# wenzhang-dev/bitcaskDB

Hardware: AMD Instinct MI355X
Metric: WAL record decode+CRC GiB/s (device-resident), 4 KiB values, 1/2/4/8 MI355X (higher is better)
Workload: dtype u8; 1 GPU; config B: 1073743514 B WAL segment per GPU, NsSize 20, 100 B keys, 4 KiB values, device-resident decode+CRC+record parse; seg_bytes=1073743514, records=253846, fragments=286402, parallelism=one independent segment per GPU x1

## Files before the change

bitcaskdb_amd/csrc/bcw_decode.hip:

```cpp
#include <hip/hip_runtime.h>

#include <cstdint>

#include "bcw_internal.h"
#include "bcw_parse.h"

namespace bcw {

enum { M_FIRST_BAD = 0,
       M_NE = 1,
       M_NFRAGS = 4, M_DONE_CRC = 5,
       M_T_CRC0 = 10, M_T_FIN = 11,
       M_ABORT = 12,
       M_BAD_CRC = 14,
       M_BAD_TYPE = 15 };

__device__ __forceinline__ uint32_t rotl32(uint32_t x, int r) { return (x << r) | (x >> (32 - r)); }

__device__ __forceinline__ void read_header(const uint8_t* __restrict__ seg, uint64_t seg_len, uint64_t off,
                                            uint32_t& crc, uint32_t& len, uint32_t& type) {
  const uint64_t a = off & ~3ull;
  uint32_t w0, w1, w2;
  if (a + 12 <= seg_len) {
    const uint32_t* q = reinterpret_cast<const uint32_t*>(seg + a);
// ... 42 lines not shown
__device__ __forceinline__ uint32_t wave_max_scan(uint32_t v, uint32_t) {
  return wave_scan_z(v, [](uint32_t x, uint32_t y) { return max(x, y); });
}
__device__ __forceinline__ uint32_t wave_or_scan(uint32_t v, uint32_t) {
  return wave_scan_z(v, [](uint32_t x, uint32_t y) { return x | y; });
}
__device__ __forceinline__ uint32_t wave_add_scan(uint32_t v, uint32_t) {
  return wave_scan_z(v, [](uint32_t x, uint32_t y) { return x + y; });
}

__device__ __forceinline__ uint32_t wg256_excl_scan(uint32_t v, uint32_t* sm4, uint32_t& total) {
  const uint32_t lane = threadIdx.x & 63u, wave = threadIdx.x >> 6;
  const uint32_t incl = wave_incl_scan_u32(v, lane);
  if (lane == 63) sm4[wave] = incl;
  __syncthreads();
  uint32_t base = 0;
  for (uint32_t k = 0; k < wave; ++k) base += sm4[k];
  total = sm4[0] + sm4[1] + sm4[2] + sm4[3];
  __syncthreads();
  return base + incl - v;
}

struct Spin {
  uint64_t t0 = 0;
  uint64_t lim = 20000000ull;
  __device__ __forceinline__ bool go(uint64_t* misc, uint32_t site) {
    const uint64_t t = wall_clock64();
    if (t0 == 0) t0 = t;
    if (t - t0 < lim &&
        __hip_atomic_load(&misc[M_ABORT], __ATOMIC_RELAXED, __HIP_MEMORY_SCOPE_AGENT) == 0ull) {
      __builtin_amdgcn_s_sleep(1);
      return true;
    }
    atomicMax(reinterpret_cast<unsigned long long*>(&misc[M_ABORT]), (unsigned long long)site);
    return false;
  }
};

constexpr int kChaseHold = 64;
constexpr uint64_t kLbAgg = 1, kLbInc = 2, kLbMask = (1ull << 38) - 1;
constexpr int kDirect = BCW_CHASE_DIRECT_MAX;

template <typename V>
__device__ __forceinline__ uint32_t chase_block(const uint8_t* __restrict__ seg, uint64_t seg_len, uint64_t boff,
                                                uint32_t bufsize, V&& visit, uint32_t h = 0, uint32_t n = 0) {
  while (h + kHdr <= bufsize) {
    uint32_t crc, len, type;
    read_header(seg, seg_len, boff + h, crc, len, type);
    const uint32_t start = h + kHdr;
    if (len > bufsize - start) len = bufsize - start;
    visit(n, start, len, crc, type);
    ++n;
    h = start + len;
  }
  return n;
}

constexpr uint32_t kRecUsual = 1u << 20, kRecAdj = 1u << 21;
__device__ __forceinline__ uint32_t check_word(uint32_t crc, uint32_t ic) { return ~rotl32(crc - 0xa282ead8u, 15) ^ ic; }
__device__ __forceinline__ void put_frag_J(Frag* __restrict__ frags, uint4* __restrict__ srec, uint64_t g,
                                           uint64_t frag_cap, uint32_t b, uint64_t boff, uint32_t start_len,
                                           uint32_t J, uint32_t type, bool adj) {
  if (g >= frag_cap) return;
  *reinterpret_cast<uint4*>(frags + g) = make_uint4(b, start_len, J, type & 0xffu);
  const uint64_t gs = boff + (start_len & 0xffffu), ge = gs + (start_len >> 16);
  const uint32_t cb = (uint32_t)(gs / kSChunk), ce = (uint32_t)(ge / kSChunk);
  const uint32_t pa = (uint32_t)(gs % kSChunk), pb = (uint32_t)(ge % kSChunk);
  const bool usual = adj && cb < ce && pb <= (uint32_t)kSChunk - 8u;
  const uint32_t e = pb + 4u, K = ((e % kSPiece) + 3u) >> 2, Lfull = e / kSPiece + (K == (uint32_t)kSPW ? 1u : 0u);
  srec[g] = make_uint4(ce, cb, J, pb | pa << 10 | (usual ? kRecUsual : 0u) | (adj ? kRecAdj : 0u) | Lfull << 22 |
                                      (K & 3u) << 29);
}
__device__ __forceinline__ void put_frag(Frag* __restrict__ frags, uint4* __restrict__ srec, uint64_t g,
                                         uint64_t frag_cap, uint32_t b, uint64_t boff, uint32_t start, uint32_t len,
                                         uint32_t crc, uint32_t type, const uint32_t* __restrict__ initc, bool adj) {
  put_frag_J(frags, srec, g, frag_cap, b, boff, start | (len << 16), check_word(crc, initc[len]), type, adj);
}

constexpr uint32_t kSumHasE = 1u << 16;

struct ClassW {
  uint64_t pw;
  uint64_t pp0, pp1;
  uint64_t p8;
  __device__ __forceinline__ uint64_t weight(uint32_t y) const {
    return (uint64_t)(65536 + 256 * (int64_t)(int8_t)(uint8_t)(pw >> (8u * y)));
  }
  __device__ __forceinline__ uint64_t prefix(uint32_t y) const {
    const uint64_t f = (y < 4u ? pp0 : pp1) >> (16u * (y & 3u));
    return (uint64_t)(65536 * (int64_t)y + 256 * (int64_t)(int16_t)(uint16_t)f);
  }
  __device__ __forceinline__ uint32_t classes_below(double x) const {
    uint32_t n = 0;
#pragma unroll
    for (uint32_t k = 1; k < 8; ++k) n += (double)prefix(k) <= x ? 1u : 0u;
    return n;
  }
};
__device__ __forceinline__ uint64_t div_floor(uint64_t a, uint64_t b, double rb) {
  uint64_t q = (uint64_t)((double)a * rb);
  while (q * b > a) --q;
  while ((q + 1) * b <= a) ++q;
  return q;
}
struct WavePart {
  ClassW cw;
  uint64_t L, nwaves, round16, den16, C;
  double rden, rC;
  __device__ __forceinline__ WavePart(const ClassW& c, uint64_t L_, uint64_t nwaves_) : cw(c), L(L_), nwaves(nwaves_) {
    const uint32_t G = (uint32_t)(nwaves / kCrcWaves);
    round16 = 16ull * cw.p8;
    den16 = round16 * (G / 8u) + 16ull * cw.prefix(G % 8u);
    C = L / 1024u;
    rden = 1.0 / (double)den16;
    rC = C ? 1.0 / (double)C : 0.0;
  }
  __device__ __forceinline__ uint64_t P(uint64_t v) const {
    if (v >= nwaves) return L;
    const uint64_t r = v / kCrcWaves;
    const uint32_t y = (uint32_t)(r % 8u);
    const uint64_t num16 = round16 * (r / 8u) + 16ull * cw.prefix(y) + cw.weight(y) * (v % kCrcWaves);
    return 1024u * div_floor(num16 * C, den16, rden);
  }
  __device__ __forceinline__ uint64_t first_at(uint64_t x) const {
    if (C == 0) return x == 0 ? 0 : nwaves;
    const uint64_t X = (x + 1023u) / 1024u, N = div_floor(X * den16 + C - 1, C, rC);
    const uint32_t q = (uint32_t)N / (uint32_t)round16;
    const uint64_t rem = N - (uint64_t)q * round16;
    uint32_t y = 0;
#pragma unroll
    for (uint32_t k = 1; k < 8; ++k) y += 16ull * cw.prefix(k) <= rem ? 1u : 0u;
    const uint64_t wy = cw.weight(y), base = 16ull * cw.prefix(y);
    const uint32_t jj = (uint32_t)(rem - base + wy - 1) / (uint32_t)wy;
    const uint64_t v = ((uint64_t)q * 8u + y) * kCrcWaves + jj;
    return v < nwaves ? v : nwaves;
  }
};

__device__ __forceinline__ ClassW class_weights(uint32_t xw) {
  ClassW c{0, 0, 0, 0};
  int64_t acc = 0;
#pragma unroll
  for (int k = 0; k < 8; ++k) {
    const int64_t d = ((int64_t)__builtin_amdgcn_readlane(xw, k) - 65536) / 256;
    c.pw |= (uint64_t)(uint8_t)(int8_t)d << (8 * k);
    if (k < 4) c.pp0 |= (uint64_t)(uint16_t)(int16_t)acc << (16 * k);
    else c.pp1 |= (uint64_t)(uint16_t)(int16_t)acc << (16 * (k - 4));
    acc += d;
  }
  c.p8 = (uint64_t)(65536 * 8 + 256 * acc);
  return c;
}

template <int ABL = 0>
__global__ __launch_bounds__(64) void k_chase(const uint8_t* __restrict__ seg, uint64_t seg_len, uint32_t start_off,
                                              uint64_t nblocks, uint32_t* __restrict__ fbase,
                                              uint32_t* __restrict__ rbase, uint2* __restrict__ bsum,
                                              Frag* __restrict__ frags, uint4* __restrict__ srec, uint64_t frag_cap,
                                              uint64_t* __restrict__ lb,
                                              uint64_t* __restrict__ lbe, uint64_t* __restrict__ misc,
                                              uint64_t epoch, const uint32_t* __restrict__ initc,
                                              uint32_t direct_max, uint64_t test_abort_wg,
                                              uint32_t* __restrict__ wstart, uint32_t nwaves,
                                              XBal* __restrict__ xb, uint32_t xb_on) {
  constexpr int kHold = (ABL & 256) ? 16 : kChaseHold;
  __shared__ uint32_t s_hold[kHold][2][64];
  __shared__ uint8_t s_type[kHold][64];
  const uint32_t lane = threadIdx.x;
  const uint32_t xw = lane < 8u ? (xb_on ? xb->w[lane] : 65536u) : 0u;
  const uint64_t tc0 = (ABL & 16) ? __builtin_amdgcn_s_memtime() : 0;
  if ((ABL & 32) && threadIdx.x == 0) lbe[4 * blockIdx.x] = wall_clock64();
  const uint64_t wg = blockIdx.x;
  if (wg >= (nblocks + 63) / 64) return;
  const uint64_t b = wg * 64 + lane;
  uint32_t bufsize = 0;
  uint64_t boff = 0;
  if (b < nblocks) {
    boff = (uint64_t)start_off + b * kBlock;
    bufsize = (uint32_t)((seg_len - boff) < kBlock ? (seg_len - boff) : kBlock);
  }
  uint32_t ne = 0, tacc = 0, tnz = 0xffffu, tst = 0, badk = 0xffffffffu;
  uint32_t hres = 0;
  const uint32_t n = chase_block(seg, seg_len, boff, bufsize,
                                 [&](uint32_t k, uint32_t start, uint32_t len, uint32_t crc, uint32_t type) {
                                   if (k < (uint32_t)kHold) {
                                     s_hold[k][0][lane] = crc;
                                     s_hold[k][1][lane] = start | (len << 16);
                                     s_type[k][lane] = (uint8_t)type;
                                   }
                                   if (k == (uint32_t)kHold - 1u) hres = start + len;
                                   if (type == BCW_RECORD_FULL || type == BCW_RECORD_LAST) {
                                     ++ne;
                                     tacc = 0;
                                     tnz = 0xffffu;
                                   } else {
                                     if (len > 0 && tnz == 0xffffu) { tnz = k; tst = start; }
                                     tacc += len;
                                     if ((type < BCW_RECORD_FULL || type > BCW_RECORD_LAST) && badk == 0xffffffffu) badk = k;
                                   }
                                 });
  const uint64_t tc1 = (ABL & 16) ? __builtin_amdgcn_s_memtime() : 0;
  if ((ABL & 32) && lane == 0) lbe[4 * wg + 1] = wall_clock64();
  if (wg == 0 && lane == 0) xb->on = xb_on;
  const uint32_t incl = wave_add_scan(n, lane);
  const uint32_t tot = __builtin_amdgcn_readlane(incl, 63);
  const uint32_t incl_e = wave_add_scan(ne, lane);
  const uint32_t tot_e = __builtin_amdgcn_readlane(incl_e, 63);
  const uint64_t tag = epoch << 40;
  const uint64_t nwg_all = (nblocks + 63) / 64;
  const bool force = wg + 1 == test_abort_wg;
  uint64_t excl = 0, excl_e = 0;
  const uint32_t nh = n < (uint32_t)kHold ? n : (uint32_t)kHold;
  auto held_checks = [&]() {
    if (ABL & 2) return;
    constexpr uint32_t kWb = 16;
    static_assert(kHold % kWb == 0, "held-header batches stay inside s_hold");
    for (uint32_t k0 = 0; k0 < nh; k0 += kWb) {
      uint32_t ic[kWb];
#pragma unroll
      for (uint32_t q = 0; q < kWb; ++q) ic[q] = initc[k0 + q < nh ? s_hold[k0 + q][1][lane] >> 16 : 0u];
#pragma unroll
      for (uint32_t q = 0; q < kWb; ++q)
        if (k0 + q < nh) s_hold[k0 + q][0][lane] = check_word(s_hold[k0 + q][0][lane], ic[q]);
    }
  };
  if (ABL & 1) {
    held_checks();
  } else if (nwg_all <= (uint64_t)direct_max) {
    if (lane == 0)
      __hip_atomic_store(&lb[wg], tag | (kLbAgg << 38) | tot | ((uint64_t)tot_e << 19), __ATOMIC_RELAXED,
                         __HIP_MEMORY_SCOPE_AGENT);
    uint64_t v[kDirect / 64];
#pragma unroll
    for (int k = 0; k < kDirect / 64; ++k) {
      const uint64_t q = lane + 64u * k;
      v[k] = q < wg ? __hip_atomic_load(&lb[q], __ATOMIC_RELAXED, __HIP_MEMORY_SCOPE_AGENT) : tag;
    }
    held_checks();
    Spin sp;
    if (force) sp.lim = 0;
    for (;;) {
      bool wait = force;
#pragma unroll
      for (int k = 0; k < kDirect / 64; ++k) wait |= (v[k] >> 40) != epoch;
      if (!__builtin_amdgcn_readfirstlane((uint32_t)(__ballot(wait) != 0ull))) break;
      if (!sp.go(misc, 9)) {
#pragma unroll
        for (int k = 0; k < kDirect / 64; ++k)
          if ((v[k] >> 40) != epoch) v[k] = 0;
        break;
      }
#pragma unroll
      for (int k = 0; k < kDirect / 64; ++k) {
        const uint64_t q = lane + 64u * k;
        if ((v[k] >> 40) != epoch) v[k] = __hip_atomic_load(&lb[q], __ATOMIC_RELAXED, __HIP_MEMORY_SCOPE_AGENT);
      }
    }
    uint64_t c = 0, ce = 0;
#pragma unroll
    for (int k = 0; k < kDirect / 64; ++k) {
      const uint64_t q = lane + 64u * k;
      if (q < wg) {
        c += v[k] & 0x7ffffu;
        ce += (v[k] >> 19) & 0x7ffffu;
      }
    }
#pragma unroll
    for (int d = 32; d >= 1; d >>= 1) {
      c += (uint64_t)__shfl_xor((long long)c, d, 64);
      ce += (uint64_t)__shfl_xor((long long)ce, d, 64);
    }
    excl = c;
    excl_e = ce;
  } else {
    const uint64_t fl = (wg == 0 ? kLbInc : kLbAgg) << 38;
    if (lane == 0) {
      __hip_atomic_store(&lb[wg], tag | fl | tot, __ATOMIC_RELAXED, __HIP_MEMORY_SCOPE_AGENT);
      __hip_atomic_store(&lbe[wg], tag | fl | tot_e, __ATOMIC_RELAXED, __HIP_MEMORY_SCOPE_AGENT);
    }
    held_checks();
    bool dn = false, de = false;
    for (uint64_t top = wg; top > 0 && !(dn && de);) {
      const uint64_t q = top - 1 - lane;
      uint64_t vn = 0, ve = 0;
      if (top > lane) {
        Spin sp;
        if (force) sp.lim = 0;
        if (!dn)
          while (((vn = __hip_atomic_load(&lb[q], __ATOMIC_RELAXED, __HIP_MEMORY_SCOPE_AGENT)) >> 40) != epoch || force)
            if (!sp.go(misc, 10)) { vn = 0; break; }
        if (!de)
          while (((ve = __hip_atomic_load(&lbe[q], __ATOMIC_RELAXED, __HIP_MEMORY_SCOPE_AGENT)) >> 40) != epoch || force)
            if (!sp.go(misc, 11)) { ve = 0; break; }
      }
      auto step = [&](uint64_t v, bool& done, uint64_t& acc) {
        if (done) return;
        const uint64_t inc = __ballot(top > lane && ((v >> 38) & 3u) == kLbInc);
        const uint32_t stop = inc ? (uint32_t)__builtin_ctzll(inc) : 64u;
        uint64_t c = (lane <= stop && top > lane) ? (v & kLbMask) : 0ull;
#pragma unroll
        for (int d = 32; d >= 1; d >>= 1) c += (uint64_t)__shfl_xor((long long)c, d, 64);
        acc += c;
        done = inc != 0;
      };
      step(vn, dn, excl);
      step(ve, de, excl_e);
      top = top > 64 ? top - 64 : 0;
    }
    if (lane == 0 && wg != 0) {
      __hip_atomic_store(&lb[wg], tag | (kLbInc << 38) | ((excl + tot) & kLbMask), __ATOMIC_RELAXED,
                         __HIP_MEMORY_SCOPE_AGENT);
      __hip_atomic_store(&lbe[wg], tag | (kLbInc << 38) | ((excl_e + tot_e) & kLbMask), __ATOMIC_RELAXED,
                         __HIP_MEMORY_SCOPE_AGENT);
    }
  }
  const uint64_t g0 = excl + incl - n;
  const uint64_t tc2 = (ABL & 16) ? __builtin_amdgcn_s_memtime() : 0;
  if ((ABL & 32) && lane == 0) lbe[4 * wg + 2] = wall_clock64();
  if (b < nblocks && !(ABL & 2)) {
    fbase[b] = (uint32_t)(g0 < 0xffffffffull ? g0 : 0xffffffffull);
    const uint64_t r0 = excl_e + incl_e - ne;
    rbase[b] = (uint32_t)(r0 < 0xffffffffull ? r0 : 0xffffffffull);
    bsum[b] = make_uint2(tacc | (tnz << 16), tst | (ne ? kSumHasE : 0u));
    if (badk != 0xffffffffu)
      atomicMin(reinterpret_cast<unsigned long long*>(&misc[M_BAD_TYPE]), (unsigned long long)(g0 + badk));
    const bool next_hdr = b + 1 < nblocks && seg_len - (boff + kBlock) >= kHdr;
    auto adj = [&](uint32_t k, uint32_t sl_k) { return k + 1u < n || (next_hdr && (sl_k & 0xffffu) + (sl_k >> 16) == kBlock); };
    const uint64_t L = seg_len - start_off, rel = boff - start_off;
    const WavePart wp(class_weights(xw), L, nwaves);
    const uint64_t span = b + 1 == nblocks ? ~0ull : (uint64_t)kBlock - 1;
    uint64_t w = wp.first_at(rel);
    uint64_t bw = wp.P(w) - rel;
    auto bounds_upto = [&](uint64_t hp, uint64_t idx) __attribute__((always_inline)) {
      const uint64_t h = hp < span ? hp : span;
      while (w <= nwaves && bw <= h) {
        wstart[w] = (uint32_t)(idx < 0xffffffffull ? idx : 0xffffffffull);
        ++w;
        bw = wp.P(w) - rel;
      }
    };
    for (uint32_t k = 0; k < nh; ++k) {
      const uint32_t sl = s_hold[k][1][lane];
      put_frag_J(frags, srec, g0 + k, frag_cap, (uint32_t)b, boff, sl, s_hold[k][0][lane], s_type[k][lane],
                 adj(k, sl));
      bounds_upto((sl & 0xffffu) - kHdr, g0 + k);
    }
    if (n > (uint32_t)kHold)
      chase_block(seg, seg_len, boff, bufsize, [&](uint32_t k, uint32_t start, uint32_t len, uint32_t crc, uint32_t type) {
        put_frag(frags, srec, g0 + k, frag_cap, (uint32_t)b, boff, start, len, crc, type, initc,
                 adj(k, start | (len << 16)));
        bounds_upto(start - kHdr, g0 + k);
      }, hres, (uint32_t)kHold);
    bounds_upto(~0ull, g0 + n);
  }
  if (ABL & 32) {
    asm volatile("s_waitcnt vmcnt(0)" ::: "memory");
    if (lane == 0) lbe[4 * wg + 3] = wall_clock64();
  }
  if (ABL & 16) {
    asm volatile("s_waitcnt vmcnt(0)" ::: "memory");
    const uint64_t tc3 = __builtin_amdgcn_s_memtime();
    if (lane == 0) {
      atomicAdd(reinterpret_cast<unsigned long long*>(&misc[7]), (unsigned long long)(tc1 - tc0));
      atomicAdd(reinterpret_cast<unsigned long long*>(&misc[8]), (unsigned long long)(tc2 - tc1));
      atomicAdd(reinterpret_cast<unsigned long long*>(&misc[9]), (unsigned long long)(tc3 - tc2));
    }
  }
  const uint64_t nwg = (nblocks + 63) / 64;
  if (lane == 63 && !(ABL & 2)) {
    const uint64_t total = excl + tot, total_e = excl_e + tot_e;
    const uint64_t be = wg * 64 + 64 < nblocks ? wg * 64 + 64 : nblocks;
    fbase[be] = (uint32_t)(total < 0xffffffffull ? total : 0xffffffffull);
    rbase[be] = (uint32_t)(total_e < 0xffffffffull ? total_e : 0xffffffffull);
    if (wg == nwg - 1) {
      misc[M_NFRAGS] = total;
      misc[M_NE] = total_e;
    }
  }
}

__device__ __forceinline__ uint32_t xor3(uint32_t a, uint32_t b, uint32_t c) {
  return __builtin_amdgcn_bitop3_b32(a, b, c, 0x96);
}
__device__ __forceinline__ uint32_t apply_fwd(const uint32_t* __restrict__ fwd, uint32_t lane, uint32_t x) {
  const uint8_t* b = reinterpret_cast<const uint8_t*>(fwd);
  const uint32_t lane4 = 4u * lane;
  auto at = [&](int i) -> uint32_t {
    const uint32_t sh = 4 * i >= 8 ? (x >> (4 * i - 8)) : (x << (8 - 4 * i));
    return *reinterpret_cast<const uint32_t*>(b + (((sh & 0xf00u) | lane4) + 4096u * (uint32_t)i));
  };
  const uint32_t r0 = at(0), r1 = at(1), r2 = at(2), r3 = at(3), r4 = at(4), r5 = at(5), r6 = at(6), r7 = at(7);
  return xor3(xor3(r0, r1, r2), xor3(r3, r4, r5), r6) ^ r7;
}
__device__ __forceinline__ uint32_t apply_op(const uint32_t* __restrict__ c, uint32_t x) {
  uint32_t r = 0;
#pragma unroll
  for (int i = 0; i < 8; ++i) r ^= c[i * 16 + ((x >> (4 * i)) & 15u)];
  return r;
}

__device__ __forceinline__ uint4 load16_slow(const uint8_t* __restrict__ seg, uint64_t seg_len, int64_t o) {
  uint64_t lo = 0, hi = 0;
#pragma unroll 1
  for (int i = 0; i < 16; ++i) {
    const int64_t q = o + i;
    const uint64_t byte = (q >= 0 && (uint64_t)q < seg_len) ? seg[q] : 0u;
    if (i < 8) lo |= byte << (8 * i); else hi |= byte << (8 * (i - 8));
  }
  return make_uint4((uint32_t)lo, (uint32_t)(lo >> 32), (uint32_t)hi, (uint32_t)(hi >> 32));
}
__device__ __forceinline__ uint4 load16_safe(const uint8_t* __restrict__ seg, uint64_t seg_len, int64_t o) {
  if (o >= 0 && (uint64_t)o + 16 <= seg_len) return *reinterpret_cast<const uint4*>(seg + o);
  return load16_slow(seg, seg_len, o);
}


template <int N>
__device__ __forceinline__ uint32_t reg_byte(const uint32_t (&h)[N], uint32_t pos) {
  uint32_t t[N];
#pragma unroll
  for (int i = 0; i < N; ++i) t[i] = h[i];
  const uint32_t wi = pos >> 2;
  int n = N;
#pragma unroll
  for (int bit = 0; bit < 6; ++bit) {
    if (n <= 1) break;
    const bool hi = (wi >> bit) & 1u;
#pragma unroll
    for (int i = 0; i < (N + 1) / 2; ++i) {
      if (i < (n + 1) / 2) t[i] = (2 * i + 1 < n) ? (hi ? t[2 * i + 1] : t[2 * i]) : t[2 * i];
    }
    n = (n + 1) / 2;
  }
  return (t[0] >> (8u * (pos & 3u))) & 0xffu;
}

constexpr int kHeadWords = 16;
constexpr int kTailWords = 8;

__device__ __attribute__((noinline)) uint32_t walk_byte(const uint8_t* __restrict__ seg, const Frag* __restrict__ frags,
                                                        uint32_t start_off, uint32_t f_first, uint32_t f_last,
                                                        uint64_t pos) {
  uint64_t beg = 0;
  for (uint32_t cf = f_first;; ++cf) {
    const Frag f = frags[cf];
    if (pos < beg + f.len || cf >= f_last)
      return seg[(uint64_t)start_off + (uint64_t)f.blk * kBlock + f.start + (pos - beg)];
    beg += f.len;
  }
}

struct RegReader {
  uint32_t h[kHeadWords];
  uint32_t t[kTailWords];
  uint32_t nhead;
  uint64_t tstart;
  uint64_t tend;
  const uint8_t* seg;
  const Frag* frags;
  uint32_t start_off;
  uint32_t f_first, f_last;
  __device__ __forceinline__ uint32_t operator()(uint64_t pos) {
    if (pos < nhead) return reg_byte(h, (uint32_t)pos);
    if (pos >= tstart && pos < tend) return reg_byte(t, (uint32_t)(pos - tstart));
    return walk_byte(seg, frags, start_off, f_first, f_last, pos);
  }
};

template <int N>
__device__ __forceinline__ void load_words(const uint8_t* __restrict__ seg, uint64_t seg_len, uint64_t base,
                                           uint32_t (&w)[N]) {
  if (base + 4u * N <= seg_len) {
#pragma unroll
    for (int k = 0; k < N / 4; ++k) {
      uint4 v;
      __builtin_memcpy(&v, seg + base + 16 * k, 16);
      w[4 * k + 0] = v.x; w[4 * k + 1] = v.y; w[4 * k + 2] = v.z; w[4 * k + 3] = v.w;
    }
  } else {
#pragma unroll
    for (int k = 0; k < N / 4; ++k) {
      const uint4 v = load16_safe(seg, seg_len, (int64_t)(base + 16 * k));
      w[4 * k + 0] = v.x; w[4 * k + 1] = v.y; w[4 * k + 2] = v.z; w[4 * k + 3] = v.w;
    }
  }
}

struct EmitArgs {
  const uint8_t* seg;
  uint64_t seg_len;
  bcw_decode_params p;
  const Frag* frags;
  const uint32_t* fbase;
  const uint32_t* rbase;
  const uint2* bsum;
  bcw_record_table tab;
  uint64_t* misc;
  uint32_t kb_flags;
  uint64_t* kb_stamps;
};


struct EmitState {
  uint64_t acc;
  int64_t nzb;
  uint32_t nzk, nzs;
  uint64_t rec;
};
__device__ __forceinline__ uint2 emit_prefetch(const EmitArgs& A, uint64_t b0, uint32_t lane) {
  return b0 > lane ? A.bsum[b0 - 1 - lane] : make_uint2(0xffff0000u, kSumHasE);
}

__device__ __forceinline__ EmitState emit_state(const EmitArgs& A, uint64_t b0, uint32_t lane, uint2 s, uint32_t rec) {
// ... 598 lines not shown
    }
  }
  __syncthreads();
  const uint64_t gw = (uint64_t)blockIdx.x * kCrcWaves + wave;
  const uint64_t f0 = wstart[gw];
  uint64_t f1 = wstart[gw + 1];
  if (f1 > frag_cap) f1 = frag_cap;
  if (f0 > f1) f1 = f0;
  const bool aborted = __builtin_amdgcn_readfirstlane(
                           (uint32_t)__hip_atomic_load(&misc[M_ABORT], __ATOMIC_RELAXED, __HIP_MEMORY_SCOPE_AGENT)) != 0u;
  if (aborted) f1 = f0;
  if (blockIdx.x == 0 && tid == 0) misc[M_T_CRC0] = wall_clock64();
  const uint32_t nfr = f1 > f0 ? (uint32_t)(f1 - f0) : 0u;
  uint64_t n_items = 0;
  auto emit_items = [&](uint64_t max_items) {
    asm volatile("" ::: "memory");
    CrcTail T;
    {
      static_assert(sizeof(CrcTail) % 4 == 0, "CrcTail words");
      const uint32_t* src = reinterpret_cast<const uint32_t*>(&s_tail);
      uint32_t* dst = reinterpret_cast<uint32_t*>(&T);
#pragma unroll
      for (int k = 0; k < (int)(sizeof(CrcTail) / 4); ++k) dst[k] = __builtin_amdgcn_readfirstlane(src[k]);
    }
    const EmitArgs& A = T.ea;
    if ((ABL & 8) || (A.kb_flags & 1u) ||
        __builtin_amdgcn_readfirstlane(
            (uint32_t)__hip_atomic_load(&T.misc[M_ABORT], __ATOMIC_RELAXED, __HIP_MEMORY_SCOPE_AGENT)) != 0u)
      return;
    const uint64_t cb0t = T.cb0, cb1t = T.cb1, fcap = T.frag_cap;
    const uint32_t cnt = (uint32_t)(cb1t - cb0t), G = gridDim.x, wg = blockIdx.x;
    const uint64_t fc0 = A.fbase[cb0t], fc1 = A.fbase[cb1t];
    const uint32_t nf_all = (uint32_t)(fc1 > fc0 ? (fc1 - fc0 < fcap ? fc1 - fc0 : fcap) : 0);
    uint32_t bpw = nf_all ? (64u * cnt) / nf_all : cnt;
    if (bpw < 1u) bpw = 1u;
    bpw = __builtin_amdgcn_readfirstlane(bpw);
    const uint32_t cq = cnt / G, cr = cnt % G;
    const uint32_t B0 = cq * wg + (cr * wg) / G, B1 = cq * (wg + 1u) + (cr * (wg + 1u)) / G;
    const uint64_t i0 = __builtin_amdgcn_readfirstlane((B0 + bpw - 1u) / bpw),
                   nitems = __builtin_amdgcn_readfirstlane((B1 + bpw - 1u) / bpw);
    auto deq = [&]() -> uint64_t {
      uint32_t j = 0;
      if (lane == 0) j = atomicAdd(&s_eq, 1u);
      j = __builtin_amdgcn_readfirstlane(j);
      return i0 + j;
    };
    uint64_t taken = 0;
    uint64_t it = deq();
    ItemMeta m = item_meta(A, it, bpw, cb0t, cb1t, lane);
    while (it < nitems) {
      ++taken;
      const EmitState es = emit_state(A, m.bb, lane, m.s, m.rec);
      const uint64_t mf1 = m.f1 < fcap ? m.f1 : fcap;
      uint64_t nx = ~0ull;
      ItemMeta mn = m;
      emit_chunks<(ABL & 4096) != 0, (ABL & 131072) != 0>(A, es, m.f0, mf1, lane, [&]() {
        if (taken < max_items) {
          nx = deq();
          mn = item_meta(A, nx, bpw, cb0t, cb1t, lane);
        }
      });
      it = nx;
      m = mn;
    }
    n_items += taken;
  };
  if (ABL & 64) emit_items(~0ull);
  if (ABL & 16384) {
    for (uint32_t q = 0; q < 4u; ++q) {
      const uint32_t a = nfr * q / 4u, b = nfr * (q + 1u) / 4u;
      stream_verify<(ABL & 8388608) != 0>(seg, seg_len, fok, srec, f0 + a, b - a, lds, lane, misc, s_rem,
                                          (wave & 3u) * 4u + (wave >> 2),
                                          reinterpret_cast<const uint8_t*>(tabs.lds_image2));
    }
  } else if (!(ABL & 32768))
    stream_verify<(ABL & 8388608) != 0>(seg, seg_len, fok, srec, f0, nfr, lds, lane, misc, s_rem,
                                        (wave & 3u) * 4u + (wave >> 2),
                                        reinterpret_cast<const uint8_t*>(tabs.lds_image2));
  __builtin_amdgcn_s_setprio(0);
  if (lane == 0) {
    atomicAdd(&s_tsum, (unsigned long long)(wall_clock64() - s_t0));
    if (atomicAdd(&s_sdone, 1u) == kCrcWaves - 1u) {
      const uint32_t c = blockIdx.x & 7u;
      __hip_atomic_fetch_add(&xb->t[c], (uint64_t)s_tsum, __ATOMIC_RELAXED, __HIP_MEMORY_SCOPE_AGENT);
      __hip_atomic_fetch_add(&xb->n[c], (uint64_t)kCrcWaves, __ATOMIC_RELAXED, __HIP_MEMORY_SCOPE_AGENT);
    }
  }
  if (ea.kb_stamps && lane == 0) {
    uint64_t* q = ea.kb_stamps + 8 * ((uint64_t)blockIdx.x * kCrcWaves + wave);
    q[0] = wall_clock64();
    q[3] = nfr;
  }
  if (!(ABL & 64)) emit_items(~0ull);
  asm volatile("" ::: "memory");
  CrcTail T;
  {
    const uint32_t* src = reinterpret_cast<const uint32_t*>(&s_tail);
    uint32_t* dst = reinterpret_cast<uint32_t*>(&T);
#pragma unroll
    for (int k = 0; k < (int)(sizeof(CrcTail) / 4); ++k) dst[k] = __builtin_amdgcn_readfirstlane(src[k]);
  }
  const EmitArgs& A = T.ea;
  if (A.kb_stamps && lane == 0) {
    uint64_t* q = A.kb_stamps + 8 * ((uint64_t)__builtin_amdgcn_workgroup_id_x() * kCrcWaves + wave);
    q[1] = wall_clock64(); q[2] = n_items;
    q[6] = __builtin_amdgcn_s_memtime();
  }
  asm volatile("s_waitcnt vmcnt(0)" ::: "memory");
  __builtin_amdgcn_fence(__ATOMIC_RELEASE, "workgroup");
  uint32_t order = 0;
  if (lane == 0) order = atomicAdd(&s_wdone, 1u);
  order = __builtin_amdgcn_readlane(order, 0);
  if (order != kCrcWaves - 1) return;
  __builtin_amdgcn_fence(__ATOMIC_ACQUIRE, "workgroup");
  uint64_t gorder = 0;
  if (lane == 0)
    gorder = __hip_atomic_fetch_add(&T.misc[M_DONE_CRC], 1ull, __ATOMIC_RELAXED, __HIP_MEMORY_SCOPE_AGENT);
  gorder = (uint64_t)__shfl((long long)gorder, 0, 64);
  if (gorder != T.nwg_total - 1u) return;
  if (lane == 0) T.misc[M_T_FIN] = wall_clock64();
  const XBalIn xin = xbal_load(xb, lane);
  finalize(A, T.nblocks, T.frag_cap, T.tail_panic, T.gen, T.res, lane);
  xbal_update(xb, lane, xin);
}

__global__ void k_export_frags(const Frag* __restrict__ frags, const uint8_t* __restrict__ fok,
                               const uint64_t* __restrict__ misc, uint64_t cap,
                               uint32_t start_off, bcw_frag_table out, const uint32_t* __restrict__ initc) {
  const uint64_t g = blockIdx.x * (uint64_t)blockDim.x + threadIdx.x;
  const uint64_t n = misc[M_NFRAGS];
  if (g >= n || g >= cap || g >= out.capacity) return;
  const Frag f = frags[g];
  out.data_off[g] = (uint64_t)start_off + (uint64_t)f.blk * kBlock + f.start;
  out.len[g] = f.len;
  const uint32_t u = ~(f.chk ^ initc[f.len]);
  out.stored_crc[g] = ((u >> 15) | (u << 17)) + 0xa282ead8u;
  out.type[g] = f.type;
  out.crc_ok[g] = fok[g];
}



hipError_t launch_decode(const uint8_t* d_seg, const bcw_decode_params& p, const bcw_record_table& t,
                         bcw_decode_result* d_result, const Tables& tabs, Scratch& s, uint64_t nblocks,
                         uint64_t gen, hipStream_t stream, int num_cus, Prof* prof) {
  Prof dummy;
  Prof& pr = prof ? *prof : dummy;
  hipEvent_t ev = nullptr;
  const uint64_t tail = (p.seg_len - p.start_off) % kBlock;
  const uint32_t tail_panic = (tail > 0 && tail < kHdr) ? 1u : 0u;
  const uint32_t nb_grid = (uint32_t)(((nblocks + 63) / 64 + 7) / 8 * 8);
  const EmitArgs ea{d_seg, p.seg_len, p, s.frags, s.fbase, s.rbase, s.bsum, t, s.misc, 0u, nullptr};
  pr.begin(K_CHASE, stream, ev);
  k_chase<0><<<nb_grid, 64, 0, stream>>>(d_seg, p.seg_len, p.start_off, nblocks, s.fbase, s.rbase, s.bsum, s.frags,
                                        s.srec, s.frag_cap, s.lb, s.lbe, s.misc, s.epoch, tabs.initc, s.chase_direct,
                                        s.test_abort_wg, s.wstart, (uint32_t)num_cus * kCrcWaves, s.xbal, s.xbal_on);
  s.test_abort_wg = 0;
  pr.end(K_CHASE, stream, ev);
  if ((++s.epoch & 0xffffffull) == 0) {
    (void)hipMemsetAsync(s.lb, 0, s.nlb * sizeof(uint64_t), stream);
    (void)hipMemsetAsync(s.lbe, 0, s.nlb * sizeof(uint64_t), stream);
    s.epoch = 1;
  }
  pr.begin(K_CRC, stream, ev);
  k_crc<0><<<(uint32_t)num_cus, kCrcThreads, 0, stream>>>(d_seg, p.seg_len, p.start_off, nblocks, s.fbase, s.fok,
                                                         s.srec, s.frag_cap, tabs, ea,
                                                         tail_panic, gen, d_result, s.misc, 0ull, nblocks,
                                                         (uint32_t)num_cus, s.wstart, s.xbal);
  pr.end(K_CRC, stream, ev);
  return hipGetLastError();
}

hipError_t launch_export_frags(const Scratch& s, const bcw_frag_table& out, uint32_t start_off, hipStream_t stream,
                               uint64_t n, const uint32_t* initc) {
  if (n == 0) return hipSuccess;
  k_export_frags<<<(uint32_t)((n + 255) / 256), 256, 0, stream>>>(s.frags, s.fok, s.misc, s.frag_cap, start_off, out,
                                                                    initc);
  return hipGetLastError();
}

}
```

Baseline: 4932 GiB/s.

## Split k_chase into specialized waves for chase, header checks and wave boundaries

k_chase grows from one wave to four per workgroup. Wave 0 chases headers and runs the decoupled look-back scan. Helper waves run the held-header CRC checks in parallel, and a dedicated wave precomputes k_crc wave-start boundaries by binary search over the held headers in LDS. Fragment emission is then striped across all waves. This aims to take the check and boundary work off the serial look-back critical path. In exchange it adds LDS, __syncthreads barriers and more threads per workgroup, which may reduce co-residency with k_crc.

```diff
diff --git a/bitcaskdb_amd/csrc/bcw_decode.hip b/bitcaskdb_amd/csrc/bcw_decode.hip
--- a/bitcaskdb_amd/csrc/bcw_decode.hip
+++ b/bitcaskdb_amd/csrc/bcw_decode.hip
@@ -218,8 +218,10 @@
   return c;
 }
 
-template <int ABL = 0>
-__global__ __launch_bounds__(64) void k_chase(const uint8_t* __restrict__ seg, uint64_t seg_len, uint32_t start_off,
+constexpr int kChaseWaves = 4;
+constexpr int kBoundHeld = 4;
+template <int ABL = 0, int WAVES = kChaseWaves>
+__global__ __launch_bounds__(WAVES * 64) void k_chase(const uint8_t* __restrict__ seg, uint64_t seg_len, uint32_t start_off,
                                               uint64_t nblocks, uint32_t* __restrict__ fbase,
                                               uint32_t* __restrict__ rbase, uint2* __restrict__ bsum,
                                               Frag* __restrict__ frags, uint4* __restrict__ srec, uint64_t frag_cap,
@@ -232,8 +234,17 @@
   constexpr int kHold = (ABL & 256) ? 16 : kChaseHold;
   __shared__ uint32_t s_hold[kHold][2][64];
   __shared__ uint8_t s_type[kHold][64];
-  const uint32_t lane = threadIdx.x;
-  const uint32_t xw = lane < 8u ? (xb_on ? xb->w[lane] : 65536u) : 0u;
+  __shared__ uint32_t s_n[64];
+  __shared__ uint64_t s_g0[64];
+  __shared__ uint16_t s_bnd[kBoundHeld * 64];
+  static_assert(WAVES >= 2 && WAVES <= 16, "wave 0 and at least one helper");
+  static_assert(sizeof(s_hold) + sizeof(s_type) + sizeof(s_n) + sizeof(s_g0) + sizeof(s_bnd) <= 44 * 1024,
+                "a k_chase workgroup fits beside a k_crc workgroup");
+  const uint32_t lane = threadIdx.x & 63u;
+  const uint32_t wv = __builtin_amdgcn_readfirstlane(threadIdx.x >> 6);
+  constexpr uint32_t kBndWave = WAVES - 1;
+  constexpr uint32_t kChkWaves = WAVES > 2 ? WAVES - 2 : 1;
+  const uint32_t xw = (wv == 0 || wv == kBndWave) && lane < 8u ? (xb_on ? xb->w[lane] : 65536u) : 0u;
   const uint64_t tc0 = (ABL & 16) ? __builtin_amdgcn_s_memtime() : 0;
   if ((ABL & 32) && threadIdx.x == 0) lbe[4 * blockIdx.x] = wall_clock64();
   const uint64_t wg = blockIdx.x;
@@ -247,184 +258,254 @@
   }
   uint32_t ne = 0, tacc = 0, tnz = 0xffffu, tst = 0, badk = 0xffffffffu;
   uint32_t hres = 0;
-  const uint32_t n = chase_block(seg, seg_len, boff, bufsize,
-                                 [&](uint32_t k, uint32_t start, uint32_t len, uint32_t crc, uint32_t type) {
-                                   if (k < (uint32_t)kHold) {
-                                     s_hold[k][0][lane] = crc;
-                                     s_hold[k][1][lane] = start | (len << 16);
-                                     s_type[k][lane] = (uint8_t)type;
-                                   }
-                                   if (k == (uint32_t)kHold - 1u) hres = start + len;
-                                   if (type == BCW_RECORD_FULL || type == BCW_RECORD_LAST) {
-                                     ++ne;
-                                     tacc = 0;
-                                     tnz = 0xffffu;
-                                   } else {
-                                     if (len > 0 && tnz == 0xffffu) { tnz = k; tst = start; }
-                                     tacc += len;
-                                     if ((type < BCW_RECORD_FULL || type > BCW_RECORD_LAST) && badk == 0xffffffffu) badk = k;
-                                   }
-                                 });
-  const uint64_t tc1 = (ABL & 16) ? __builtin_amdgcn_s_memtime() : 0;
-  if ((ABL & 32) && lane == 0) lbe[4 * wg + 1] = wall_clock64();
-  if (wg == 0 && lane == 0) xb->on = xb_on;
-  const uint32_t incl = wave_add_scan(n, lane);
-  const uint32_t tot = __builtin_amdgcn_readlane(incl, 63);
-  const uint32_t incl_e = wave_add_scan(ne, lane);
-  const uint32_t tot_e = __builtin_amdgcn_readlane(incl_e, 63);
+  uint32_t n = 0, incl = 0, tot = 0, incl_e = 0, tot_e = 0;
+  uint64_t tc1 = 0;
   const uint64_t tag = epoch << 40;
   const uint64_t nwg_all = (nblocks + 63) / 64;
+  const bool direct = nwg_all <= (uint64_t)direct_max;
   const bool force = wg + 1 == test_abort_wg;
+  if (wv == 0) {
+    n = chase_block(seg, seg_len, boff, bufsize,
+                    [&](uint32_t k, uint32_t start, uint32_t len, uint32_t crc, uint32_t type) {
+                      if (k < (uint32_t)kHold) {
+                        s_hold[k][0][lane] = crc;
+                        s_hold[k][1][lane] = start | (len << 16);
+                        s_type[k][lane] = (uint8_t)type;
+                      }
+                      if (k == (uint32_t)kHold - 1u) hres = start + len;
+                      if (type == BCW_RECORD_FULL || type == BCW_RECORD_LAST) {
+                        ++ne;
+                        tacc = 0;
+                        tnz = 0xffffu;
+                      } else {
+                        if (len > 0 && tnz == 0xffffu) { tnz = k; tst = start; }
+                        tacc += len;
+                        if ((type < BCW_RECORD_FULL || type > BCW_RECORD_LAST) && badk == 0xffffffffu) badk = k;
+                      }
+                    });
+    s_n[lane] = n;
+    tc1 = (ABL & 16) ? __builtin_amdgcn_s_memtime() : 0;
+    if ((ABL & 32) && lane == 0) lbe[4 * wg + 1] = wall_clock64();
+    if (wg == 0 && lane == 0) xb->on = xb_on;
+    incl = wave_add_scan(n, lane);
+    tot = __builtin_amdgcn_readlane(incl, 63);
+    incl_e = wave_add_scan(ne, lane);
+    tot_e = __builtin_amdgcn_readlane(incl_e, 63);
+    if (!(ABL & 1) && lane == 0) {
+      if (direct) {
+        __hip_atomic_store(&lb[wg], tag | (kLbAgg << 38) | tot | ((uint64_t)tot_e << 19), __ATOMIC_RELAXED,
+                           __HIP_MEMORY_SCOPE_AGENT);
+      } else {
+        const uint64_t fl = (wg == 0 ? kLbInc : kLbAgg) << 38;
+        __hip_atomic_store(&lb[wg], tag | fl | tot, __ATOMIC_RELAXED, __HIP_MEMORY_SCOPE_AGENT);
+        __hip_atomic_store(&lbe[wg], tag | fl | tot_e, __ATOMIC_RELAXED, __HIP_MEMORY_SCOPE_AGENT);
+      }
+    }
+  }
+  __syncthreads();
   uint64_t excl = 0, excl_e = 0;
-  const uint32_t nh = n < (uint32_t)kHold ? n : (uint32_t)kHold;
-  auto held_checks = [&]() {
-    if (ABL & 2) return;
-    constexpr uint32_t kWb = 16;
-    static_assert(kHold % kWb == 0, "held-header batches stay inside s_hold");
-    for (uint32_t k0 = 0; k0 < nh; k0 += kWb) {
-      uint32_t ic[kWb];
-#pragma unroll
-      for (uint32_t q = 0; q < kWb; ++q) ic[q] = initc[k0 + q < nh ? s_hold[k0 + q][1][lane] >> 16 : 0u];
-#pragma unroll
-      for (uint32_t q = 0; q < kWb; ++q)
-        if (k0 + q < nh) s_hold[k0 + q][0][lane] = check_word(s_hold[k0 + q][0][lane], ic[q]);
-    }
+  const uint32_t nh = min(s_n[lane], (uint32_t)kHold);
+  const uint64_t L = seg_len - start_off;
+  const uint64_t rel0 = wg * 64u * (uint64_t)kBlock;
+  const bool last_wg = wg * 64u + 64u >= nblocks;
+  const uint32_t nbl = last_wg ? (uint32_t)(nblocks - wg * 64u) : 64u;
+  auto resolve = [&](const WavePart& wp, uint64_t w, uint32_t& e) __attribute__((always_inline)) -> uint32_t {
+    if (w > nwaves) return 0u;
+    const uint64_t p = wp.P(w) - rel0;
+    if (!last_wg && p > 64u * (uint64_t)kBlock - 1u) return 0u;
+    const uint32_t bl = min((uint32_t)min(p / kBlock, (uint64_t)63u), nbl - 1u);
+    const uint64_t bw = p - (uint64_t)bl * kBlock;
+    const uint32_t nb = s_n[bl], nhb = min(nb, (uint32_t)kHold);
+    uint32_t cnt = 0;
+#pragma unroll
+    for (uint32_t s = kHold; s >= 1u; s >>= 1) {
+      const uint32_t i = cnt + s - 1u;
+      if (i < nhb && (uint64_t)((s_hold[i][1][bl] & 0xffffu) - kHdr) < bw) cnt += s;
+    }
+    if (cnt == (uint32_t)kHold && nb > (uint32_t)kHold) return 2u;
+    e = bl | cnt << 8;
+    return 1u;
   };
-  if (ABL & 1) {
-    held_checks();
-  } else if (nwg_all <= (uint64_t)direct_max) {
-    if (lane == 0)
-      __hip_atomic_store(&lb[wg], tag | (kLbAgg << 38) | tot | ((uint64_t)tot_e << 19), __ATOMIC_RELAXED,
-                         __HIP_MEMORY_SCOPE_AGENT);
-    uint64_t v[kDirect / 64];
-#pragma unroll
-    for (int k = 0; k < kDirect / 64; ++k) {
-      const uint64_t q = lane + 64u * k;
-      v[k] = q < wg ? __hip_atomic_load(&lb[q], __ATOMIC_RELAXED, __HIP_MEMORY_SCOPE_AGENT) : tag;
-    }
-    held_checks();
-    Spin sp;
-    if (force) sp.lim = 0;
-    for (;;) {
-      bool wait = force;
-#pragma unroll
-      for (int k = 0; k < kDirect / 64; ++k) wait |= (v[k] >> 40) != epoch;
-      if (!__builtin_amdgcn_readfirstlane((uint32_t)(__ballot(wait) != 0ull))) break;
-      if (!sp.go(misc, 9)) {
-#pragma unroll
-        for (int k = 0; k < kDirect / 64; ++k)
-          if ((v[k] >> 40) != epoch) v[k] = 0;
-        break;
-      }
+  uint64_t w_lo = 0;
+  uint32_t bnd_done = 0;
+  if (wv == 0) {
+    if (ABL & 1) {
+    } else if (direct) {
+      uint64_t v[kDirect / 64];
 #pragma unroll
       for (int k = 0; k < kDirect / 64; ++k) {
         const uint64_t q = lane + 64u * k;
-        if ((v[k] >> 40) != epoch) v[k] = __hip_atomic_load(&lb[q], __ATOMIC_RELAXED, __HIP_MEMORY_SCOPE_AGENT);
-      }
-    }
-    uint64_t c = 0, ce = 0;
-#pragma unroll
-    for (int k = 0; k < kDirect / 64; ++k) {
-      const uint64_t q = lane + 64u * k;
-      if (q < wg) {
-        c += v[k] & 0x7ffffu;
-        ce += (v[k] >> 19) & 0x7ffffu;
-      }
-    }
-#pragma unroll
-    for (int d = 32; d >= 1; d >>= 1) {
-      c += (uint64_t)__shfl_xor((long long)c, d, 64);
-      ce += (uint64_t)__shfl_xor((long long)ce, d, 64);
-    }
-    excl = c;
-    excl_e = ce;
-  } else {
-    const uint64_t fl = (wg == 0 ? kLbInc : kLbAgg) << 38;
-    if (lane == 0) {
-      __hip_atomic_store(&lb[wg], tag | fl | tot, __ATOMIC_RELAXED, __HIP_MEMORY_SCOPE_AGENT);
-      __hip_atomic_store(&lbe[wg], tag | fl | tot_e, __ATOMIC_RELAXED, __HIP_MEMORY_SCOPE_AGENT);
-    }
-    held_checks();
-    bool dn = false, de = false;
-    for (uint64_t top = wg; top > 0 && !(dn && de);) {
-      const uint64_t q = top - 1 - lane;
-      uint64_t vn = 0, ve = 0;
-      if (top > lane) {
-        Spin sp;
-        if (force) sp.lim = 0;
-        if (!dn)
-          while (((vn = __hip_atomic_load(&lb[q], __ATOMIC_RELAXED, __HIP_MEMORY_SCOPE_AGENT)) >> 40) != epoch || force)
-            if (!sp.go(misc, 10)) { vn = 0; break; }
-        if (!de)
-          while (((ve = __hip_atomic_load(&lbe[q], __ATOMIC_RELAXED, __HIP_MEMORY_SCOPE_AGENT)) >> 40) != epoch || force)
-            if (!sp.go(misc, 11)) { ve = 0; break; }
-      }
-      auto step = [&](uint64_t v, bool& done, uint64_t& acc) {
-        if (done) return;
-        const uint64_t inc = __ballot(top > lane && ((v >> 38) & 3u) == kLbInc);
-        const uint32_t stop = inc ? (uint32_t)__builtin_ctzll(inc) : 64u;
-        uint64_t c = (lane <= stop && top > lane) ? (v & kLbMask) : 0ull;
-#pragma unroll
-        for (int d = 32; d >= 1; d >>= 1) c += (uint64_t)__shfl_xor((long long)c, d, 64);
-        acc += c;
-        done = inc != 0;
-      };
-      step(vn, dn, excl);
-      step(ve, de, excl_e);
-      top = top > 64 ? top - 64 : 0;
-    }
-    if (lane == 0 && wg != 0) {
-      __hip_atomic_store(&lb[wg], tag | (kLbInc << 38) | ((excl + tot) & kLbMask), __ATOMIC_RELAXED,
-                         __HIP_MEMORY_SCOPE_AGENT);
-      __hip_atomic_store(&lbe[wg], tag | (kLbInc << 38) | ((excl_e + tot_e) & kLbMask), __ATOMIC_RELAXED,
-                         __HIP_MEMORY_SCOPE_AGENT);
-    }
-  }
-  const uint64_t g0 = excl + incl - n;
+        v[k] = q < wg ? __hip_atomic_load(&lb[q], __ATOMIC_RELAXED, __HIP_MEMORY_SCOPE_AGENT) : tag;
+      }
+      Spin sp;
+      if (force) sp.lim = 0;
+      for (;;) {
+        bool wait = force;
+#pragma unroll
+        for (int k = 0; k < kDirect / 64; ++k) wait |= (v[k] >> 40) != epoch;
+        if (!__builtin_amdgcn_readfirstlane((uint32_t)(__ballot(wait) != 0ull))) break;
+        if (!sp.go(misc, 9)) {
+#pragma unroll
+          for (int k = 0; k < kDirect / 64; ++k)
+            if ((v[k] >> 40) != epoch) v[k] = 0;
+          break;
+        }
+#pragma unroll
+        for (int k = 0; k < kDirect / 64; ++k) {
+          const uint64_t q = lane + 64u * k;
+          if ((v[k] >> 40) != epoch) v[k] = __hip_atomic_load(&lb[q], __ATOMIC_RELAXED, __HIP_MEMORY_SCOPE_AGENT);
+        }
+      }
+      uint64_t c = 0, ce = 0;
+#pragma unroll
+      for (int k = 0; k < kDirect / 64; ++k) {
+        const uint64_t q = lane + 64u * k;
+        if (q < wg) {
+          c += v[k] & 0x7ffffu;
+          ce += (v[k] >> 19) & 0x7ffffu;
+        }
+      }
+#pragma unroll
+      for (int d = 32; d >= 1; d >>= 1) {
+        c += (uint64_t)__shfl_xor((long long)c, d, 64);
+        ce += (uint64_t)__shfl_xor((long long)ce, d, 64);
+      }
+      excl = c;
+      excl_e = ce;
+    } else {
+      bool dn = false, de = false;
+      for (uint64_t top = wg; top > 0 && !(dn && de);) {
+        const uint64_t q = top - 1 - lane;
+        uint64_t vn = 0, ve = 0;
+        if (top > lane) {
+          Spin sp;
+          if (force) sp.lim = 0;
+          if (!dn)
+            while (((vn = __hip_atomic_load(&lb[q], __ATOMIC_RELAXED, __HIP_MEMORY_SCOPE_AGENT)) >> 40) != epoch ||
+                   force)
+              if (!sp.go(misc, 10)) { vn = 0; break; }
+          if (!de)
+            while (((ve = __hip_atomic_load(&lbe[q], __ATOMIC_RELAXED, __HIP_MEMORY_SCOPE_AGENT)) >> 40) != epoch ||
+                   force)
+              if (!sp.go(misc, 11)) { ve = 0; break; }
+        }
+        auto step = [&](uint64_t v, bool& done, uint64_t& acc) {
+          if (done) return;
+          const uint64_t inc = __ballot(top > lane && ((v >> 38) & 3u) == kLbInc);
+          const uint32_t stop = inc ? (uint32_t)__builtin_ctzll(inc) : 64u;
+          uint64_t c = (lane <= stop && top > lane) ? (v & kLbMask) : 0ull;
+#pragma unroll
+          for (int d = 32; d >= 1; d >>= 1) c += (uint64_t)__shfl_xor((long long)c, d, 64);
+          acc += c;
+          done = inc != 0;
+        };
+        step(vn, dn, excl);
+        step(ve, de, excl_e);
+        top = top > 64 ? top - 64 : 0;
+      }
+      if (lane == 0 && wg != 0) {
+        __hip_atomic_store(&lb[wg], tag | (kLbInc << 38) | ((excl + tot) & kLbMask), __ATOMIC_RELAXED,
+                           __HIP_MEMORY_SCOPE_AGENT);
+        __hip_atomic_store(&lbe[wg], tag | (kLbInc << 38) | ((excl_e + tot_e) & kLbMask), __ATOMIC_RELAXED,
+                           __HIP_MEMORY_SCOPE_AGENT);
+      }
+    }
+    s_g0[lane] = excl + incl - n;
+  } else if (!(ABL & 2)) {
+    if (wv <= kChkWaves) {
+      constexpr uint32_t kWb = 16;
+      static_assert(kHold % kWb == 0, "held-header batches stay inside s_hold");
+      for (uint32_t k0 = kWb * (wv - 1u); k0 < nh; k0 += kWb * kChkWaves) {
+        uint32_t ic[kWb];
+#pragma unroll
+        for (uint32_t q = 0; q < kWb; ++q) ic[q] = initc[k0 + q < nh ? s_hold[k0 + q][1][lane] >> 16 : 0u];
+#pragma unroll
+        for (uint32_t q = 0; q < kWb; ++q)
+          if (k0 + q < nh) s_hold[k0 + q][0][lane] = check_word(s_hold[k0 + q][0][lane], ic[q]);
+      }
+    }
+    if (wv == kBndWave) {
+      const WavePart wp(class_weights(xw), L, nwaves);
+      w_lo = wp.first_at(rel0);
+      for (; bnd_done < (uint32_t)kBoundHeld; ++bnd_done) {
+        uint32_t e = 0;
+        const uint32_t r = resolve(wp, w_lo + 64u * bnd_done + lane, e);
+        if (__ballot(r != 0u) == 0ull) { bnd_done |= 0x100u; break; }
+        s_bnd[64u * bnd_done + lane] = (uint16_t)(r == 1u ? e : 0xffffu);
+      }
+    }
+  }
   const uint64_t tc2 = (ABL & 16) ? __builtin_amdgcn_s_memtime() : 0;
-  if ((ABL & 32) && lane == 0) lbe[4 * wg + 2] = wall_clock64();
+  if ((ABL & 32) && threadIdx.x == 0) lbe[4 * wg + 2] = wall_clock64();
+  __syncthreads();
   if (b < nblocks && !(ABL & 2)) {
-    fbase[b] = (uint32_t)(g0 < 0xffffffffull ? g0 : 0xffffffffull);
-    const uint64_t r0 = excl_e + incl_e - ne;
-    rbase[b] = (uint32_t)(r0 < 0xffffffffull ? r0 : 0xffffffffull);
-    bsum[b] = make_uint2(tacc | (tnz << 16), tst | (ne ? kSumHasE : 0u));
-    if (badk != 0xffffffffu)
-      atomicMin(reinterpret_cast<unsigned long long*>(&misc[M_BAD_TYPE]), (unsigned long long)(g0 + badk));
+    const uint64_t g0 = s_g0[lane];
+    n = s_n[lane];
+    if (wv == 0) {
+      fbase[b] = (uint32_t)(g0 < 0xffffffffull ? g0 : 0xffffffffull);
+      const uint64_t r0 = excl_e + incl_e - ne;
+      rbase[b] = (uint32_t)(r0 < 0xffffffffull ? r0 : 0xffffffffull);
+      bsum[b] = make_uint2(tacc | (tnz << 16), tst | (ne ? kSumHasE : 0u));
+      if (badk != 0xffffffffu)
+        atomicMin(reinterpret_cast<unsigned long long*>(&misc[M_BAD_TYPE]), (unsigned long long)(g0 + badk));
+    }
     const bool next_hdr = b + 1 < nblocks && seg_len - (boff + kBlock) >= kHdr;
     auto adj = [&](uint32_t k, uint32_t sl_k) { return k + 1u < n || (next_hdr && (sl_k & 0xffffu) + (sl_k >> 16) == kBlock); };
-    const uint64_t L = seg_len - start_off, rel = boff - start_off;
-    const WavePart wp(class_weights(xw), L, nwaves);
-    const uint64_t span = b + 1 == nblocks ? ~0ull : (uint64_t)kBlock - 1;
-    uint64_t w = wp.first_at(rel);
-    uint64_t bw = wp.P(w) - rel;
-    auto bounds_upto = [&](uint64_t hp, uint64_t idx) __attribute__((always_inline)) {
-      const uint64_t h = hp < span ? hp : span;
-      while (w <= nwaves && bw <= h) {
-        wstart[w] = (uint32_t)(idx < 0xffffffffull ? idx : 0xffffffffull);
-        ++w;
-        bw = wp.P(w) - rel;
-      }
-    };
-    for (uint32_t k = 0; k < nh; ++k) {
+    for (uint32_t k = wv; k < nh; k += (uint32_t)WAVES) {
       const uint32_t sl = s_hold[k][1][lane];
       put_frag_J(frags, srec, g0 + k, frag_cap, (uint32_t)b, boff, sl, s_hold[k][0][lane], s_type[k][lane],
                  adj(k, sl));
-      bounds_upto((sl & 0xffffu) - kHdr, g0 + k);
-    }
-    if (n > (uint32_t)kHold)
+    }
+    if (wv == 0 && n > (uint32_t)kHold) {
+      const uint64_t rel = boff - start_off;
+      const WavePart wp(class_weights(xw), L, nwaves);
+      const uint64_t span = b + 1 == nblocks ? ~0ull : (uint64_t)kBlock - 1;
+      uint64_t w = wp.first_at(rel + (s_hold[kHold - 1][1][lane] & 0xffffu) - kHdr + 1u);
+      uint64_t bw = wp.P(w) - rel;
+      auto bounds_upto = [&](uint64_t hp, uint64_t idx) __attribute__((always_inline)) {
+        const uint64_t h = hp < span ? hp : span;
+        while (w <= nwaves && bw <= h) {
+          wstart[w] = (uint32_t)(idx < 0xffffffffull ? idx : 0xffffffffull);
+          ++w;
+          bw = wp.P(w) - rel;
+        }
+      };
       chase_block(seg, seg_len, boff, bufsize, [&](uint32_t k, uint32_t start, uint32_t len, uint32_t crc, uint32_t type) {
         put_frag(frags, srec, g0 + k, frag_cap, (uint32_t)b, boff, start, len, crc, type, initc,
                  adj(k, start | (len << 16)));
         bounds_upto(start - kHdr, g0 + k);
       }, hres, (uint32_t)kHold);
-    bounds_upto(~0ull, g0 + n);
-  }
+      bounds_upto(~0ull, g0 + n);
+    }
+  }
+  if (wv == kBndWave && !(ABL & 2)) {
+    auto put = [&](uint64_t w, uint32_t e) {
+      const uint64_t idx = s_g0[e & 0xffu] + (e >> 8);
+      wstart[w] = (uint32_t)(idx < 0xffffffffull ? idx : 0xffffffffull);
+    };
+    for (uint32_t i = 0; i < (bnd_done & 0xffu); ++i) {
+      const uint32_t e = s_bnd[64u * i + lane];
+      if (e != 0xffffu) put(w_lo + 64u * i + lane, e);
+    }
+    if (!(bnd_done & 0x100u)) {
+      const WavePart wp(class_weights(xw), L, nwaves);
+      for (uint64_t base = w_lo + 64u * (uint32_t)kBoundHeld;; base += 64u) {
+        uint32_t e = 0;
+        const uint32_t r = resolve(wp, base + lane, e);
+        if (__ballot(r != 0u) == 0ull) break;
+        if (r == 1u) put(base + lane, e);
+      }
+    }
+  }
+  if (ABL & 48) {
+    asm volatile("s_waitcnt vmcnt(0)" ::: "memory");
+    __syncthreads();
+  }
+  if (wv != 0) return;
   if (ABL & 32) {
-    asm volatile("s_waitcnt vmcnt(0)" ::: "memory");
     if (lane == 0) lbe[4 * wg + 3] = wall_clock64();
   }
   if (ABL & 16) {
-    asm volatile("s_waitcnt vmcnt(0)" ::: "memory");
     const uint64_t tc3 = __builtin_amdgcn_s_memtime();
     if (lane == 0) {
       atomicAdd(reinterpret_cast<unsigned long long*>(&misc[7]), (unsigned long long)(tc1 - tc0));
@@ -1329,7 +1410,7 @@
   const uint32_t nb_grid = (uint32_t)(((nblocks + 63) / 64 + 7) / 8 * 8);
   const EmitArgs ea{d_seg, p.seg_len, p, s.frags, s.fbase, s.rbase, s.bsum, t, s.misc, 0u, nullptr};
   pr.begin(K_CHASE, stream, ev);
-  k_chase<0><<<nb_grid, 64, 0, stream>>>(d_seg, p.seg_len, p.start_off, nblocks, s.fbase, s.rbase, s.bsum, s.frags,
+  k_chase<0><<<nb_grid, kChaseWaves * 64, 0, stream>>>(d_seg, p.seg_len, p.start_off, nblocks, s.fbase, s.rbase, s.bsum, s.frags,
                                         s.srec, s.frag_cap, s.lb, s.lbe, s.misc, s.epoch, tabs.initc, s.chase_direct,
                                         s.test_abort_wg, s.wstart, (uint32_t)num_cus * kCrcWaves, s.xbal, s.xbal_on);
   s.test_abort_wg = 0;
```

Measured after the change: 5020 GiB/s, median of 6. 1.02x the previous value.
